# WISDEM/RAFT

Hardware: AMD Instinct MI355X
Metric: design-case-frequency solves/sec (whole node) (higher is better)
Workload: dtype f64

## Files before the change

### raft_amd/csrc/raftx_geom.h

```cpp
#pragma once

#define MP_N 24
#define MH_N 48
#define MI_N 48

__host__ __device__ inline void derive_design_tables(const double *strips, int64_t i0, int64_t i1, double *dsv,
                                                     int *dsf) {
    int64_t s = i0;
    while (s < i1) {
        int64_t e = s + 1;
        double proj[64];
        int np = 0;
        while (e < i1 && (e - s) < 64) {
            const double *pr = strips + (size_t)(e - 1) * NF, *cr = strips + (size_t)e * NF;
            bool same = true;
            double dv[3], pj = 0.0;
            for (int j = 0; j < 3; j++) {
                same = same && (pr[RAFTX_F_Q + j] == cr[RAFTX_F_Q + j]);
                dv[j] = cr[RAFTX_F_X + j] - pr[RAFTX_F_X + j];
                pj += dv[j] * cr[RAFTX_F_Q + j];
            }
            if (!same || !(pj > 0.0) || !(fabs(pj) <= 1.797e308)) break;
            double perp2 = 0.0, scale = 1.0;
            for (int j = 0; j < 3; j++) {
// ... 616 lines not shown
            for (int c = 0; c < 3; c++) {
                ra[c] = rA[c] + q[c] * a[RAFTX_GS_S];
                rb[c] = rA[c] + q[c] * b[RAFTX_GS_S];
            }
            const double aD1 = circ ? a[RAFTX_GS_D] : a[RAFTX_GS_D + 1], bD1 = circ ? b[RAFTX_GS_D] : b[RAFTX_GS_D + 1];
            if (ra[2] * rb[2] <= 0) {
                const double t = (0 - ra[2]);
                double xWP = ra[0] + t * (rb[0] - ra[0]) / (rb[2] - ra[2]);
                double yWP = ra[1] + t * (rb[1] - ra[1]) / (rb[2] - ra[2]);
                const double w0 = b[RAFTX_GS_D] + t * (a[RAFTX_GS_D] - b[RAFTX_GS_D]) / (rb[2] - ra[2]);
                const double w1 = bD1 + t * (aD1 - bD1) / (rb[2] - ra[2]);
                double AWP, IxWP, IyWP;
                if (circ) {
                    AWP = (M_PI / 4) * w0 * w0;
                    IxWP = IyWP = (M_PI / 64) * w0 * w0 * w0 * w0;
                } else {
                    AWP = w0 * w1;
                    const double Ix = (1.0 / 12) * w0 * w1 * w1 * w1, Iy = (1.0 / 12) * w0 * w0 * w0 * w1;
                    IxWP = R[0][0] * Ix * R[0][0] + R[0][1] * Iy * R[0][1];
                    IyWP = R[1][0] * Ix * R[1][0] + R[1][1] * Iy * R[1][1];
                }
                const double LWP = fabs(ra[2] / cosPhi);
                double V, hc;
                geom_frustum(a[RAFTX_GS_D], aD1, w0, w1, circ, LWP, V, hc);
                double M = 0.0;
                if (circ) M = -rg * M_PI * (w0 * w0 / 32 * (2.0 + tanPhi * tanPhi) + 0.5 * (ra[2] / cosPhi) * (ra[2] / cosPhi)) * sinPhi;
                const double Fz = rg * V;
                const double ex = ra[0] - rA[0], ey = ra[1] - rA[1];
                F[2] += Fz;
                F[3] += ey * Fz;
                F[4] += -ex * Fz;
                F[3] += M * (-sinBeta);
                F[4] += M * cosBeta;
                xWP -= rA[0];
                yWP -= rA[1];
                C[2 * 6 + 2] += rg * AWP / cosPhi;
                C[2 * 6 + 3] += rg * (-AWP * yWP);
                C[2 * 6 + 4] += rg * (AWP * xWP);
                C[3 * 6 + 2] += rg * (-AWP * yWP);
                C[3 * 6 + 3] += rg * (IxWP + AWP * yWP * yWP);
                C[3 * 6 + 4] += rg * (AWP * xWP * yWP);
                C[4 * 6 + 2] += rg * (AWP * xWP);
                C[4 * 6 + 3] += rg * (AWP * xWP * yWP);
                C[4 * 6 + 4] += rg * (IyWP + AWP * xWP * xWP);
                double rc[3];
                for (int c = 0; c < 3; c++) rc[c] = ra[c] + q[c] * hc;
                C[3 * 6 + 3] += rg * V * (rc[2] - rA[2]);
                C[4 * 6 + 4] += rg * V * (rc[2] - rA[2]);
                C[3 * 6 + 5] += -rg * V * (rc[0] - rA[0]);
                C[4 * 6 + 5] += -rg * V * (rc[1] - rA[1]);
                Vt += V;
                for (int c = 0; c < 3; c++) rcV[c] += rc[c] * V;
                AWPm = AWP;
            } else if (ra[2] <= 0 && rb[2] <= 0) {
                double V, hc;
                geom_frustum(a[RAFTX_GS_D], aD1, b[RAFTX_GS_D], bD1, circ, b[RAFTX_GS_S] - a[RAFTX_GS_S], V, hc);
                double rc[3], rr[3];
                for (int c = 0; c < 3; c++) { rc[c] = ra[c] + q[c] * hc; rr[c] = rc[c] - rA[c]; }
                const double Fz = rg * V;
                F[2] += Fz;
                F[3] += rr[1] * Fz;
                F[4] += -rr[0] * Fz;
                C[3 * 6 + 3] += rg * V * rr[2];
                C[4 * 6 + 4] += rg * V * rr[2];
                C[3 * 6 + 5] += -rg * V * rr[0];
                C[4 * 6 + 5] += -rg * V * rr[1];
                Vt += V;
                for (int c = 0; c < 3; c++) rcV[c] += rc[c] * V;
            }
        }
    }
    if (geom_along(rA[2], rB[2], b[RAFTX_GS_S], L) < 0) wet++;
    double *mh = A.mhyd + (size_t)m * MH_N, *mi = A.minert + (size_t)m * MI_N;
    if (!nostatic) {
        for (int i = 0; i < 36; i++) mh[i] = C[i];
        for (int i = 0; i < 6; i++) mh[36 + i] = F[i];
        mh[42] = Vt; mh[43] = rcV[0]; mh[44] = rcV[1]; mh[45] = rcV[2]; mh[46] = AWPm; mh[47] = 0.0;
    }
    int code = 0;
    if (!nostatic) {
        GInertia J;
        geom_inertia_init(J);
        geom_load_row(gs, 0, b);
        for (int i = 1; i < n; i++) {
#pragma unroll
            for (int f = 0; f < RAFTX_GS_N; f++) a[f] = b[f];
            geom_load_row(gs, i, b);
            geom_inertia_section(J, a, b, circ, rho_shell, trim, 0.0, rA, q, p1, p2);
        }
        const int ncap = A.capOff ? (int)(co1 - co0) : 0;
        const double *gc = A.capOff ? A.caps + (size_t)co0 * RAFTX_GC_N : nullptr;
        code = geom_inertia_caps_finish(J, gs, n, gc, ncap, circ, rho_shell, rA, q, p1, p2, A.g, mi);
    }
    double *mp = A.mpose + (size_t)m * MP_N;
    for (int i = 0; i < 3; i++) {
        mp[i] = rA0[i]; mp[3 + i] = rA[i]; mp[6 + i] = q[i]; mp[9 + i] = p1[i]; mp[12 + i] = p2[i];
    }
    mp[15] = R[0][0]; mp[16] = R[0][1]; mp[17] = R[1][0]; mp[18] = R[1][1]; mp[19] = L;
    const int wetm = ((flags & RAFTX_GM_FLAG_MCF) && circ && !(flags & RAFTX_GM_FLAG_POTMOD)) ? wet : 0;
    A.cnt[m] = wet;
    A.cntm[m] = wetm;
    if (wet) atomicAdd(reinterpret_cast<unsigned long long *>(A.off + d + 1), (unsigned long long)wet);
    if (wetm) atomicAdd(reinterpret_cast<unsigned long long *>(A.cmoff + d + 1), (unsigned long long)wetm);
    if (nostatic) {
        for (int i = 0; i < MH_N; i++) mh[i] = 0.0;
        for (int i = 0; i < MI_N; i++) mi[i] = 0.0;
        return;
    }
    if (code) {
        for (int i = 0; i < MI_N; i++) mi[i] = 0.0;
        atomicCAS(A.err, 0, (int)(m + 1));
    }
}

__global__ void k_geom_trim(GeomArgs A) {
    GEOM_NOFMA
    if (A.err[2] | A.err[3]) return;
    const int d = blockIdx.x * blockDim.x + threadIdx.x;
    if (d >= A.nDesign) return;
    double mass = A.M0[(size_t)d * 36], V = 0.0, vol = 0.0;
    for (int64_t m = A.mo(d); m < A.mo(d + 1); m++) {
        mass += A.minert[(size_t)m * MI_N + 36];
        vol += A.minert[(size_t)m * MI_N + 47];
        V += A.mhyd[(size_t)m * MH_N + 42];
    }
    if (!(vol > 0.0)) {
        A.drho[d] = 0.0;
        atomicCAS(A.err + 1, 0, d + 1);
        return;
    }
    const double sumFz = -mass * A.g + V * A.rho * A.g + (A.Fz ? A.Fz[d] : 0.0);
    A.drho[d] = sumFz / A.g / vol;
}
__global__ __launch_bounds__(128) void k_geom_reinertia(GeomArgs A) {
    GEOM_NOFMA
    if (A.err[2] | A.err[3]) return;
    const int64_t m = geom_member_of_thread(A);
    if (m < 0) return;
    const double *gm = A.gm + (size_t)m * RAFTX_GM_N;
    if ((int)gm[RAFTX_GM_FLAGS] & RAFTX_GM_FLAG_NOSTATIC) return;
    const double *gs = A.gs + (size_t)A.so(m) * RAFTX_GS_N;
    const int n = (int)(A.so(m + 1) - A.so(m));
    const double *mp = A.mpose + (size_t)m * MP_N;
    const int ncap = A.capOff ? (int)(A.co(m + 1) - A.co(m)) : 0;
    const double *gc = A.capOff ? A.caps + (size_t)A.co(m) * RAFTX_GC_N : nullptr;
    double *mi = A.minert + (size_t)m * MI_N;
    if (geom_member_inertia(gm, gs, n, gc, ncap, mp + 3, mp + 6, mp + 9, mp + 12, A.g, true, A.drho[A.mdesign[m]], mi))
        for (int i = 0; i < MI_N; i++) mi[i] = 0.0;
}

#define GSCAN_CH 4096
template <int T>
__global__ __launch_bounds__(T) void k_geom_scan_t(GeomArgs A) {
    __shared__ long long part[2][17];
    __shared__ unsigned buf[2][GSCAN_CH];
    const int t = threadIdx.x;
    const int n = A.nDesign;
    constexpr int PER = GSCAN_CH / T;
    long long carrya = 0, carryb = 0, mx = 0;
    for (int c0 = 0; c0 < n; c0 += GSCAN_CH) {
        const int cn = (n - c0 < GSCAN_CH) ? n - c0 : GSCAN_CH;
        for (int i = t; i < GSCAN_CH; i += T) {
            long long va = 0, vb = 0;
            if (i < cn) { va = A.off[c0 + i + 1]; vb = A.cmoff[c0 + i + 1]; }
            buf[0][i] = (unsigned)va;
            buf[1][i] = (unsigned)vb;
            mx = va > mx ? va : mx;
        }
        __syncthreads();
        long long a = 0, b = 0;
        for (int i = 0; i < PER; i++) { a += buf[0][t * PER + i]; b += buf[1][t * PER + i]; }
        const int lane = t & 63, wv = t >> 6;
        long long ia = a, ib = b;
        for (int o = 1; o < 64; o <<= 1) {
            const long long ua = __shfl_up(ia, o, 64), ub = __shfl_up(ib, o, 64);
            if (lane >= o) { ia += ua; ib += ub; }
        }
        if (lane == 63) { part[0][wv] = ia; part[1][wv] = ib; }
        __syncthreads();
        long long ra = carrya, rb = carryb, sa = 0, sb = 0;
        for (int i = 0; i < T / 64; i++) {
            if (i < wv) { ra += part[0][i]; rb += part[1][i]; }
            sa += part[0][i]; sb += part[1][i];
        }
        ra += ia - a;
        rb += ib - b;
        for (int i = 0; i < PER; i++) {
            ra += buf[0][t * PER + i];
            rb += buf[1][t * PER + i];
            buf[0][t * PER + i] = (unsigned)ra;
            buf[1][t * PER + i] = (unsigned)rb;
        }
        __syncthreads();
        for (int i = t; i < cn; i += T) {
            const long long va = buf[0][i], vb = buf[1][i];
            A.off[c0 + i + 1] = va;
            A.cmoff[c0 + i + 1] = vb;
            if (A.hostOut) A.hostOut[8 + c0 + i + 1] = va;
        }
        carrya += sa;
        carryb += sb;
        __syncthreads();
    }
    if (mx) atomicMax(reinterpret_cast<unsigned long long *>(A.tot + 2), (unsigned long long)mx);
    __syncthreads();
    if (t == 0) {
        A.off[0] = 0;
        A.cmoff[0] = 0;
        A.tot[0] = carrya;
        A.tot[1] = carryb;
        if (A.hostOut) {
            A.hostOut[0] = carrya;
            A.hostOut[1] = carryb;
            A.hostOut[2] = A.tot[2];
            int *e = reinterpret_cast<int *>(A.hostOut + 3);
            e[0] = A.err[0]; e[1] = A.err[1]; e[2] = A.err[2]; e[3] = A.err[3];
            A.hostOut[8] = 0;
        }
    }
}
__global__ __launch_bounds__(64) void k_geom_mcf(GeomArgs A, int64_t nRows) {
    GEOM_NOFMA
    const int64_t row = blockIdx.x;
    const int iw = blockIdx.y * blockDim.x + threadIdx.x;
    if (row >= nRows || iw >= A.nw) return;
    const double R = A.mcfaux[row * 3], Ca1 = A.mcfaux[row * 3 + 1], Ca2 = A.mcfaux[row * 3 + 2];
    const double k = A.k[iw];
    const double Tr = M_PI / 5 / R;
    double ramp;
    if (k <= 0.0) ramp = 0.0;
    else if (k < Tr) ramp = 0.5 * (1 - cos(M_PI * k / Tr));
    else ramp = 1.0;
    double cr = 0.0, ci = 0.0;
    if (ramp != 0.0) {
        const double x = k * R;
        const double hr = 0.5 * (j0(x) - jn(2, x)), hi = 0.5 * (y0(x) - yn(2, x));
        const double den = M_PI * (x * x);
        const double mag = den * (hr * hr + hi * hi);
        cr = 4.0 * hi / mag;
        ci = 4.0 * hr / mag;
    }
    A.cm[((size_t)row * 2 + 0) * A.nw + iw] = cplx{cr * ramp + (1.0 + Ca1) * (1 - ramp), ci * ramp};
    A.cm[((size_t)row * 2 + 1) * A.nw + iw] = cplx{cr * ramp + (1.0 + Ca2) * (1 - ramp), ci * ramp};
}


__device__ inline void geom_reduce_matrix(const double *C, const double (&a)[3], double *out) {
    GEOM_NOFMA
    const double H[3][3] = {{0, a[2], -a[1]}, {-a[2], 0, a[0]}, {a[1], -a[0], 0}};
    double t12[3][3], t21[3][3];
    for (int i = 0; i < 3; i++)
        for (int j = 0; j < 3; j++) {
            double s12 = C[i * 6 + 3 + j], s21 = C[(3 + i) * 6 + j];
            for (int l = 0; l < 3; l++) {
                s12 += C[i * 6 + l] * H[l][j];
                s21 += H[l][i] * C[l * 6 + j];
            }
            t12[i][j] = s12;
            t21[i][j] = s21;
        }
    for (int i = 0; i < 3; i++)
        for (int j = 0; j < 3; j++) {
            out[i * 6 + j] += C[i * 6 + j];
            out[i * 6 + 3 + j] += t12[i][j];
            out[(3 + i) * 6 + j] += t21[i][j];
            double s = C[(3 + i) * 6 + 3 + j];
            for (int l = 0; l < 3; l++) s += H[l][i] * t12[l][j] + C[(3 + i) * 6 + l] * H[l][j];
            out[(3 + i) * 6 + 3 + j] += s;
        }
}
__device__ inline void geom_reduce_vector(const double *W, const double (&a)[3], const double *arm0, const double (&th)[3],
                                          double *Wout, double *Cout) {
    GEOM_NOFMA
    Wout[0] += W[0]; Wout[1] += W[1]; Wout[2] += W[2];
    Wout[3] += W[3] + (a[1] * W[2] - a[2] * W[1]);
    Wout[4] += W[4] + (a[2] * W[0] - a[0] * W[2]);
    Wout[5] += W[5] + (a[0] * W[1] - a[1] * W[0]);
    for (int j = 0; j < 3; j++) {
        double tj[3] = {th[0], th[1], th[2]};
        tj[j] += 1.0;
        const double dA[3] = {arm0[0] + (tj[1] * a[2] - tj[2] * a[1]) - a[0], arm0[1] + (tj[2] * a[0] - tj[0] * a[2]) - a[1],
                              arm0[2] + (tj[0] * a[1] - tj[1] * a[0]) - a[2]};
        Cout[3 * 6 + 3 + j] -= dA[1] * W[2] - dA[2] * W[1];
        Cout[4 * 6 + 3 + j] -= dA[2] * W[0] - dA[0] * W[2];
        Cout[5 * 6 + 3 + j] -= dA[0] * W[1] - dA[1] * W[0];
    }
}

__device__ constexpr int DS_SRC[DS_N] = {
    -1, -1, RAFTX_F_MCF, -1,
    RAFTX_F_X, RAFTX_F_X + 1, RAFTX_F_X + 2,
    -2, -3, -4,
    RAFTX_F_AX, RAFTX_F_AX + 1, RAFTX_F_AX + 2,
    RAFTX_F_Q, RAFTX_F_Q + 1, RAFTX_F_Q + 2,
    RAFTX_F_P1, RAFTX_F_P1 + 1, RAFTX_F_P1 + 2,
    RAFTX_F_P2, RAFTX_F_P2 + 1, RAFTX_F_P2 + 2,
    RAFTX_F_IQ, RAFTX_F_IP1, RAFTX_F_IP2, RAFTX_F_AI, RAFTX_F_RHOV,
    RAFTX_F_DQ, RAFTX_F_DP1, RAFTX_F_DP2, RAFTX_F_DEND, -1};
static_assert(DS_MCF == 2 && DS_X == 4 && DS_U == 7 && DS_A == 10 && DS_Q == 13 && DS_P1 == 16 && DS_P2 == 19 &&
              DS_IQ == 22 && DS_DQ == 27 && DS_N == 32, "DS_SRC follows the device record layout");
#define GD_ROW (NF + 1)
#define GD_GM_N 3
#define GD_MP_N 13
#ifdef GEOM_PHASE_TIMING
__device__ unsigned long long geom_phase_cycles[10];
#define GEOM_PHASE(i)                                                                                   \
    do {                                                                                                \
        __syncthreads();                                                                                \
        const unsigned long long now_ = wall_clock64();                                                 \
        if (threadIdx.x == 0) atomicAdd(&geom_phase_cycles[i], now_ - tphase_);                         \
        tphase_ = now_;                                                                                 \
    } while (0)
#define GEOM_PHASE_BEGIN unsigned long long tphase_ = wall_clock64();
#else
#define GEOM_PHASE(i)
#define GEOM_PHASE_BEGIN
#endif
#ifndef GD_T
#define GD_T 128
#endif
static_assert(GD_T % 64 == 0 && GD_T % DS_N == 0 && GD_T <= 256, "k_geom_design: whole wavefronts, a lane keeps its record field");
template <bool ABI, bool ADDUP>
__device__ __forceinline__ void geom_design_block(const GeomArgs &A, const int d, double *gd_lds, int *wcnt) {
    GEOM_NOFMA
    const int lane = threadIdx.x;
    const int64_t i0 = A.off[d], i1 = A.off[d + 1];
    const int S = (int)(i1 - i0);
    double *rec = gd_lds;
    double *pjv = rec + (size_t)S * GD_ROW, *unv = pjv + S;
    int *okv = reinterpret_cast<int *>(unv + S), *rsv = okv + S, *mfl = rsv + S;
    GEOM_PHASE_BEGIN
    {
        const int64_t m0 = A.mo(d), m1 = A.mo(d + 1);
        const int nMem = (int)(m1 - m0);
        const int64_t s0 = A.so(m0);
        const int nSta = (int)(A.so(m1) - s0);
        int *mcum = mfl + S;
        int *mbase = mcum + nSta + 2 * nMem;
        int *ssta = mbase + nMem + 1;
        double *sgm = reinterpret_cast<double *>(okv + (((int)(ssta - okv) + nMem + 2) & ~1));
        double *sgs = sgm + (size_t)nMem * GD_GM_N;
        double *smp = sgs + (size_t)nSta * RAFTX_GS_N;
        {
            const double *g0 = A.gm + (size_t)m0 * RAFTX_GM_N, *g1 = A.gs + (size_t)s0 * RAFTX_GS_N, *g2 = A.mpose + (size_t)m0 * MP_N;
            const int n0 = nMem * GD_GM_N, n01 = n0 + nSta * RAFTX_GS_N, total = n01 + nMem * GD_MP_N;
            constexpr int SU = 10;
            const int64_t so_lane = lane <= nMem ? A.so(m0 + lane) : s0;
            for (int base = 0; base < total; base += SU * GD_T) {
                double v[SU];
#pragma unroll
                for (int u = 0; u < SU; u++) {
                    const int idx = base + u * GD_T + lane;
                    const double *src;
                    if (idx < n0) {
                        const int row = idx / GD_GM_N, col = idx % GD_GM_N;
                        src = g0 + (size_t)row * RAFTX_GM_N + (col == 0 ? RAFTX_GM_DLSMAX : (col == 1 ? RAFTX_GM_SHAPE : RAFTX_GM_FLAGS));
                    } else if (idx < n01) {
                        src = g1 + (idx - n0);
                    } else {
                        const int k = idx - n01, row = k / GD_MP_N, col = k % GD_MP_N;
                        src = g2 + (size_t)row * MP_N + (col < 12 ? 3 + col : 19);
                    }
                    v[u] = idx < total ? *src : 0.0;
                }
#pragma unroll
                for (int u = 0; u < SU; u++) {
                    const int idx = base + u * GD_T + lane;
                    if (idx < total) sgm[idx] = v[u];
                }
            }
            if (lane <= nMem) mbase[lane] = ssta[lane] = (int)(so_lane - s0);
            for (int mi = lane + GD_T; mi <= nMem; mi += GD_T) mbase[mi] = ssta[mi] = (int)(A.so(m0 + mi) - s0);
        }
        __syncthreads();
        for (int u = lane; u < nSta + nMem; u += GD_T) {
            int mi = 0;
            while (mi + 1 < nMem && mbase[mi + 1] + mi + 1 <= u) mi++;
            const int sta0 = mbase[mi], n = mbase[mi + 1] - sta0, g = u - (sta0 + mi);
            int cntg = 1;
            if (g > 0 && g < n) {
                const double *gs = sgs + (size_t)sta0 * RAFTX_GS_N;
                cntg = geom_interval_strips(gs[(size_t)g * RAFTX_GS_N + RAFTX_GS_S] - gs[(size_t)(g - 1) * RAFTX_GS_N + RAFTX_GS_S],
                                            sgm[(size_t)mi * GD_GM_N]);
            }
            mcum[sta0 + 2 * mi + g + 1] = cntg;
        }
        __syncthreads();
        for (int mi = lane; mi < nMem; mi += GD_T) {
            const int n = ssta[mi + 1] - ssta[mi];
            int *cum = mcum + ssta[mi] + 2 * mi;
            int a = 0;
            cum[0] = 0;
            for (int g = 0; g <= n; g++) { a += cum[g + 1]; cum[g + 1] = a; }
            mbase[mi + 1] = a;
        }
        __syncthreads();
        if (lane == 0) {
            int a = 0;
            mbase[0] = 0;
            for (int mi = 0; mi < nMem; mi++) { a += mbase[mi + 1]; mbase[mi + 1] = a; }
        }
        __syncthreads();
        const int total = mbase[nMem];
        GEOM_PHASE(0);
        const double rho = A.rho, cdrag = sqrt(8 / M_PI);
        double rP[3] = {0, 0, 0};
        if (A.pose)
            for (int i = 0; i < 3; i++) rP[i] = A.pose[(size_t)d * 6 + i];
        int nwet = 0;
        for (int t0 = 0; t0 < total; t0 += GD_T) {
            const int t = t0 + lane;
            const bool act = t < total;
            const int tq = act ? t : 0;
            int mi = 0;
            while (mi + 1 < nMem && mbase[mi + 1] <= tq) mi++;
            const int64_t m = m0 + mi;
            const int tt = tq - mbase[mi];
            const int n = ssta[mi + 1] - ssta[mi];
            const int *cum = mcum + ssta[mi] + 2 * mi;
            const double *gm = sgm + (size_t)mi * GD_GM_N;
            const double *gs = sgs + (size_t)ssta[mi] * RAFTX_GS_N;
            const double *mp = smp + (size_t)mi * GD_MP_N;
            const bool circ = gm[1] != 0.0;
            const int flags = (int)gm[2];
            const bool potMod = flags & RAFTX_GM_FLAG_POTMOD;
            const bool mcf = (flags & RAFTX_GM_FLAG_MCF) && circ && !potMod;
            const double L = mp[12];
            double rA[3], rB[3], q[3], p1[3], p2[3], armN[3];
            for (int i = 0; i < 3; i++) {
                rA[i] = mp[i]; q[i] = mp[3 + i]; p1[i] = mp[6 + i]; p2[i] = mp[9 + i];
                rB[i] = rA[i] + L * q[i];
                armN[i] = rA[i] - rP[i];
            }
            int g = 0;
            while (g < n && cum[g + 1] <= tt) g++;
            const int j = tt - cum[g];
            const int nsub = (g > 0 && g < n) ? cum[g + 1] - cum[g] : 1;
            GStrip st = geom_strip(gs, n, g, j, nsub, circ);
            double r[3];
            for (int c = 0; c < 3; c++) r[c] = geom_along(rA[c], rB[c], st.ls, L);
            const bool wet = act && (r[2] < 0);
            const GLocate at = geom_locate(st.ls, gs, n);
            const unsigned long long mask = __ballot(wet);
            const int wv = lane >> 6, ln = lane & 63;
            if (ln == 0) wcnt[wv] = __popcll(mask);
            __syncthreads();
            int before = 0, all = 0;
            for (int w = 0; w < GD_T / 64; w++) {
                before += w < wv ? wcnt[w] : 0;
                all += wcnt[w];
            }
            const int pos = nwet + before + __popcll(mask & ((1ull << ln) - 1ull));
            nwet += all;
            __syncthreads();
            if (!wet || pos >= S) continue;
            double *row = rec + (size_t)pos * GD_ROW;
            for (int c = 0; c < NF; c++) row[c] = 0.0;
            for (int c = 0; c < 3; c++) {
                row[RAFTX_F_X + c] = r[c];
                row[RAFTX_F_AX + c] = (r[c] - rA[c]) + armN[c];
                row[RAFTX_F_Q + c] = q[c];
                row[RAFTX_F_P1 + c] = p1[c];
                row[RAFTX_F_P2 + c] = p2[c];
            }
            row[RAFTX_F_CIRC] = circ ? 1.0 : 0.0;
            row[RAFTX_F_MCF] = -1.0;
            row[26] = (double)mi;
            row[27] = (double)tt;
            const double ds0 = st.ds0, ds1 = st.ds1, dr0 = st.drs0, dr1 = st.drs1, dls = st.dls;
            if (!potMod) {
                double v_i, v_end, a_i;
                if (circ) {
                    v_i = 0.25 * M_PI * ds0 * ds0 * dls;
                    const double a3 = ds0 + dr0, b3 = ds0 - dr0;
                    v_end = M_PI / 12.0 * fabs(a3 * a3 * a3 - b3 * b3 * b3);
                    a_i = M_PI * ds0 * dr0;
                } else {
                    v_i = ds0 * ds1 * dls;
                    const double ma = 0.5 * ((ds0 + dr0) + (ds1 + dr1)), mb = 0.5 * ((ds0 - dr0) + (ds1 - dr1));
                    v_end = M_PI / 12.0 * (ma * ma * ma - mb * mb * mb);
                    a_i = (ds0 + dr0) * (ds1 + dr1) - (ds0 - dr0) * (ds1 - dr1);
                }
                if (r[2] + 0.5 * dls > 0) v_i = v_i * (0.5 * dls - r[2]) / dls;
                const double Ca1 = geom_interp_at(at, st.ls, gs, RAFTX_GS_CA + 1), Ca2 = geom_interp_at(at, st.ls, gs, RAFTX_GS_CA + 2);
                const double CaE = geom_interp_at(at, st.ls, gs, RAFTX_GS_CA + 3);
                row[RAFTX_F_IQ] = rho * v_end * CaE;
                row[RAFTX_F_AI] = a_i;
                row[RAFTX_F_RHOV] = rho * v_i;
                row[RAFTX_F_AP1] = rho * v_i * Ca1;
                row[RAFTX_F_AP2] = rho * v_i * Ca2;
                if (mcf) {
                    int64_t cmbase = A.cmoff[d], cmrow0 = cmbase;
                    int wet0 = 0;
                    for (int64_t mm = m0; mm < m; mm++) { cmrow0 += A.cntm[mm]; wet0 += A.cnt[mm]; }
                    const int posm = pos - wet0;
                    row[RAFTX_F_MCF] = (double)((cmrow0 - cmbase) + posm);
                    double *ax = A.mcfaux + (size_t)(cmrow0 + posm) * 3;
                    ax[0] = ds0 / 2; ax[1] = Ca1; ax[2] = Ca2;
                } else {
                    row[RAFTX_F_IP1] = rho * v_i * (1.0 + Ca1);
                    row[RAFTX_F_IP2] = rho * v_i * (1.0 + Ca2);
                }
            }
            double a_q, a_p1, a_p2, a_end;
            if (circ) {
                a_q = M_PI * ds0 * dls; a_p1 = ds0 * dls; a_p2 = ds0 * dls; a_end = fabs(M_PI * ds0 * dr0);
            } else {
                a_q = 2 * (ds0 + ds0) * dls; a_p1 = ds0 * dls; a_p2 = ds1 * dls;
                a_end = fabs((ds0 + dr0) * (ds1 + dr1) - (ds0 - dr0) * (ds1 - dr1));
            }
            row[RAFTX_F_DQ] = cdrag * 0.5 * rho * a_q * geom_interp_at(at, st.ls, gs, RAFTX_GS_CD + 0);
            row[RAFTX_F_DP1] = cdrag * 0.5 * rho * a_p1 * geom_interp_at(at, st.ls, gs, RAFTX_GS_CD + 1);
            row[RAFTX_F_DP2] = cdrag * 0.5 * rho * a_p2 * geom_interp_at(at, st.ls, gs, RAFTX_GS_CD + 2);
            row[RAFTX_F_DEND] = cdrag * 0.5 * rho * a_end * geom_interp_at(at, st.ls, gs, RAFTX_GS_CD + 3);
        }
        __syncthreads();
        GEOM_PHASE(1);
        if constexpr (ABI) {
            double *abi = A.abi + (size_t)i0 * NF;
            for (int t = lane; t < S * NF; t += GD_T) abi[t] = rec[(t / NF) * GD_ROW + (t % NF)];
        }
    }
    __syncthreads();
    GEOM_PHASE(2);
    for (int t = lane; t < S; t += GD_T) {
        bool pass = false;
        double pj = 0.0;
        const double *pr = rec + (size_t)(t > 0 ? t - 1 : 0) * GD_ROW, *cr = rec + (size_t)t * GD_ROW;
        double pq[3], cq[3], px[3], cx[3];
        for (int j = 0; j < 3; j++) {
            pq[j] = pr[RAFTX_F_Q + j]; cq[j] = cr[RAFTX_F_Q + j]; px[j] = pr[RAFTX_F_X + j]; cx[j] = cr[RAFTX_F_X + j];
        }
        if (t > 0) {
            bool same = true;
            double dv[3];
            for (int j = 0; j < 3; j++) {
                same = same && (pq[j] == cq[j]);
                dv[j] = cx[j] - px[j];
                pj += dv[j] * cq[j];
            }
            if (same && (pj > 0.0) && (fabs(pj) <= 1.797e308)) {
                double perp2 = 0.0, scale = 1.0;
                for (int j = 0; j < 3; j++) {
                    double tt = dv[j] - pj * cq[j];
                    perp2 += tt * tt;
                    scale += fabs(cx[j]);
                }
                pass = !(sqrt(perp2) > 1e-10 * scale);
            }
        }
        okv[t] = pass ? 1 : 0;
        pjv[t] = pj;
    }
    __syncthreads();
    bool serial = S > GD_T;
    if (!serial) {
        const int wv = lane >> 6, ln = lane & 63;
        const bool st = lane < S && (lane == 0 || !okv[lane]);
        const unsigned long long mask = __ballot(st);
        if (ln == 0) wcnt[wv] = mask ? wv * 64 + 63 - __builtin_clzll(mask) : -1;
        if (st) reinterpret_cast<unsigned long long *>(unv)[lane] = 0x7ff0000000000000ull;
        __syncthreads();
        const unsigned long long below = mask & (ln == 63 ? ~0ull : ((2ull << ln) - 1ull));
        int s = below ? wv * 64 + 63 - __builtin_clzll(below) : -1;
        for (int w = wv - 1; w >= 0 && s < 0; w--) s = wcnt[w];
        if (lane < S) {
            rsv[lane] = s;
            if (!st) atomicMin(reinterpret_cast<unsigned long long *>(unv) + s, (unsigned long long)__double_as_longlong(pjv[lane]));
        }
        serial = __syncthreads_or(lane < S && lane - s >= 64) != 0;
        if (!serial && st && reinterpret_cast<unsigned long long *>(unv)[lane] == 0x7ff0000000000000ull) unv[lane] = 0.0;
    }
    if (serial && lane == 0) {
        int s = 0;
        double unit = 0.0;
        for (int t = 0; t < S; t++) {
            if (t == 0 || !okv[t] || (t - s) >= 64) {
                if (t > 0) unv[s] = unit;
                s = t;
                unit = 0.0;
            } else {
                const double pj = pjv[t];
                unit = (unit == 0.0 || pj < unit) ? pj : unit;
            }
            rsv[t] = s;
        }
        if (S > 0) unv[s] = unit;
    }
    __syncthreads();
    for (int t = lane; t < S; t += GD_T) {
        const int s = rsv[t];
        const double unit = unv[s];
        const double *cr = rec + (size_t)t * GD_ROW, *pr = rec + (size_t)(t > 0 ? t - 1 : 0) * GD_ROW;
        double cX[3], cQ[3], cP1[3], cP2[3], cA[3], pX[3], pP1[3], pP2[3], pA[3];
        for (int j = 0; j < 3; j++) {
            cX[j] = cr[RAFTX_F_X + j]; cQ[j] = cr[RAFTX_F_Q + j]; cP1[j] = cr[RAFTX_F_P1 + j]; cP2[j] = cr[RAFTX_F_P2 + j];
            cA[j] = cr[RAFTX_F_AX + j];
            pX[j] = pr[RAFTX_F_X + j]; pP1[j] = pr[RAFTX_F_P1 + j]; pP2[j] = pr[RAFTX_F_P2 + j]; pA[j] = pr[RAFTX_F_AX + j];
        }
        const double cCirc = cr[RAFTX_F_CIRC], cMcf = cr[RAFTX_F_MCF], pCirc = pr[RAFTX_F_CIRC], pMcf = pr[RAFTX_F_MCF];
        const double pjt = pjv[t];
        int m = 0;
        if (t > s && unit > 0.0) {
            double ratio = pjt / unit;
            int mi = (int)floor(ratio + 0.5);
            if (mi >= 1 && mi <= 2 && fabs(ratio - mi) < 1e-9) {
                bool ok = true;
                for (int j = 0; j < 3; j++) {
                    double pred = pX[j] + (double)mi * unit * cQ[j];
                    if (fabs(pred - cX[j]) > 1e-10 * (1.0 + fabs(cX[j]))) ok = false;
                }
                if (ok) m = mi;
            }
        }
        if (m != 0) {
            for (int j = 0; j < 3; j++)
                if (pP1[j] != cP1[j] || pP2[j] != cP2[j]) m = 0;
            if ((pCirc != 0.0) != (cCirc != 0.0)) m = 0;
            if ((pMcf >= 0.0) != (cMcf >= 0.0)) m = 0;
            for (int j = 0; j < 3; j++) {
                const double da = cA[j] - pA[j], dx = cX[j] - pX[j];
                if (!(fabs(da - dx) <= 1e-9 * (1.0 + fabs(cX[j]) + fabs(cA[j])))) m = 0;
            }
        }
        int fl = m | (cCirc != 0.0 ? DSI_CIRC : 0);
        if (fabs(cP1[0]) < 1e-15 && fabs(cP1[1]) < 1e-15 && fabs(cP2[2]) < 1e-15) fl |= DSI_AXAL;
        if (fabs(cQ[0]) < 1e-15 && fabs(cQ[1]) < 1e-15 && fabs(cP1[2]) < 1e-15 && fabs(cP2[2]) < 1e-15)
            fl |= DSI_VAX;
        A.dsi[(size_t)i0 + t] = fl;
    }
    GEOM_PHASE(3);
    {
        double *dso = A.ds + (size_t)i0 * DS_N;
        const int j = lane % DS_N, f = DS_SRC[j], nT = S * DS_N;
        constexpr int DU = 4;
        for (int t0 = lane; t0 < nT; t0 += DU * GD_T) {
          double vv[DU];
#pragma unroll
          for (int u = 0; u < DU; u++) {
            const int t = t0 + u * GD_T;
            const int i = t < nT ? t / DS_N : 0;
            const double *cr = rec + (size_t)i * GD_ROW;
            double v = 0.0;
            if (f >= 0) v = cr[f];
            else if (f <= -2) v = unv[rsv[i]] * cr[RAFTX_F_Q + (-2 - f)];
            if (t < nT && j == DS_MCF && v >= 0.0) {
                const double *ax0 = A.mcfaux + (size_t)A.cmoff[d] * 3, *axm = ax0 + (size_t)v * 3;
                const int mrow = (int)v;
                for (int r = 0; r < mrow; r++)
                    if (ax0[r * 3] == axm[0] && ax0[r * 3 + 1] == axm[1] && ax0[r * 3 + 2] == axm[2]) {
                        v = (double)r;
                        break;
                    }
            }
            vv[u] = v;
          }
#pragma unroll
          for (int u = 0; u < DU; u++) {
            const int t = t0 + u * GD_T;
            if (t < nT) dso[t] = vv[u];
          }
        }
    }
    GEOM_PHASE(4);
    constexpr int GV = 21;
    for (int t0 = 0; t0 < S; t0 += GD_T) {
        const int t = t0 + lane;
        double gv[GV];
        if (t < S) {
            const double *cr = rec + (size_t)t * GD_ROW;
            const double ax = cr[RAFTX_F_AX], ay = cr[RAFTX_F_AX + 1], az = cr[RAFTX_F_AX + 2];
            const double cs[3] = {cr[RAFTX_F_AP1], cr[RAFTX_F_AP2], cr[RAFTX_F_IQ]};
            const int fs[3] = {RAFTX_F_P1, RAFTX_F_P2, RAFTX_F_Q};
            for (int tt = 0; tt < 3; tt++) {
                const double nx = cr[fs[tt]], ny = cr[fs[tt] + 1], nz = cr[fs[tt] + 2];
                gv[tt * 7] = cs[tt];
                gv[tt * 7 + 1] = nx; gv[tt * 7 + 2] = ny; gv[tt * 7 + 3] = nz;
                gv[tt * 7 + 4] = ay * nz - az * ny;
                gv[tt * 7 + 5] = az * nx - ax * nz;
                gv[tt * 7 + 6] = ax * ny - ay * nx;
            }
        }
        __syncthreads();
        if (t < S)
            for (int e = 0; e < GV; e++) rec[(size_t)t * GV + e] = gv[e];
    }
    __syncthreads();
    GEOM_PHASE(5);
    {
        const int k3 = lane / 36, e = lane % 36, i = e / 6, j = e % 6;
        double am = 0.0;
        if (k3 < 3) {
            const int lo = (int)(((long long)S * k3) / 3), hi = (int)(((long long)S * (k3 + 1)) / 3);
            for (int s = lo; s < hi; s++) {
                const double *g = rec + (size_t)s * GV;
                for (int tt = 0; tt < 3; tt++) am += g[tt * 7] * g[tt * 7 + 1 + i] * g[tt * 7 + 1 + j];
            }
        }
        __syncthreads();
        if (k3 < 3) rec[lane] = am;
        __syncthreads();
        if (lane < 36) {
            am = (rec[lane] + rec[36 + lane]) + rec[72 + lane];
            const size_t o = (size_t)d * 36 + lane;
            A.A[o] = am;
            if constexpr (ADDUP) {
                double m0 = A.M0[o], c0 = A.C0[o];
                if (A.add_mask & RAFTX_ADD_MORISON) m0 += am;
                if (A.add_mask & RAFTX_ADD_HYDROSTATIC) c0 += A.Ch[o];
                if (A.add_mask & RAFTX_ADD_INERTIA) { m0 += A.Ms[o]; c0 += A.Cs[o]; }
                A.M0[o] = m0;
                A.C0[o] = c0;
            }
        }
    }
    GEOM_PHASE(6);
    (void)mfl;
}
__global__ __launch_bounds__(GD_T) void k_geom_design(GeomArgs A) {
    extern __shared__ double gd_lds[];
    __shared__ int wcnt[GD_T / 64];
    if ((int)blockIdx.x >= A.nDesign) return;
    if (A.abi) geom_design_block<true, false>(A, (int)blockIdx.x, gd_lds, wcnt);
    else if (A.addup_in_design) geom_design_block<false, true>(A, (int)blockIdx.x, gd_lds, wcnt);
    else geom_design_block<false, false>(A, (int)blockIdx.x, gd_lds, wcnt);
}
__global__ void k_geom_addup(GeomArgs A) {
    const size_t o = (size_t)blockIdx.x * blockDim.x + threadIdx.x;
    if (o >= (size_t)A.nDesign * 36) return;
    if (A.add_mask & RAFTX_ADD_MORISON) A.M0[o] += A.A[o];
    if (A.add_mask & RAFTX_ADD_HYDROSTATIC) A.C0[o] += A.Ch[o];
    if (A.add_mask & RAFTX_ADD_INERTIA) { A.M0[o] += A.Ms[o]; A.C0[o] += A.Cs[o]; }
}
static size_t geom_design_lds(int maxS, int maxSta, int maxMem) {
    const size_t S = (size_t)(maxS > 0 ? maxS : 1);
    return sizeof(double) * (S * GD_ROW + 2 * S) + sizeof(int) * (3 * S + (size_t)maxSta + 3 * (size_t)maxMem + 1) + 16 +
           sizeof(int) * ((size_t)maxMem + 4) +
           sizeof(double) * ((size_t)maxMem * (GD_GM_N + GD_MP_N) + (size_t)maxSta * RAFTX_GS_N);
}

__global__ __launch_bounds__(64) void k_geom_reduce(GeomArgs A) {
    GEOM_NOFMA
    const int t = blockIdx.x * blockDim.x + threadIdx.x;
    const int d = t / 3, role = t % 3;
    if (d >= A.nDesign) return;
    double th[3] = {0, 0, 0}, rP[3] = {0, 0, 0};
    if (A.pose)
        for (int i = 0; i < 3; i++) { rP[i] = A.pose[(size_t)d * 6 + i]; th[i] = A.pose[(size_t)d * 6 + 3 + i]; }
    double out[36], Wv[6] = {0, 0, 0, 0, 0, 0}, sc0 = 0.0, sc1 = 0.0, sr[3] = {0, 0, 0};
    for (int i = 0; i < 36; i++) out[i] = 0.0;
    for (int64_t m = A.mo(d); m < A.mo(d + 1); m++) {
        const double *mp = A.mpose + (size_t)m * MP_N, *mh = A.mhyd + (size_t)m * MH_N, *mi = A.minert + (size_t)m * MI_N;
        const double a[3] = {mp[3] - rP[0], mp[4] - rP[1], mp[5] - rP[2]};
        double C[36];
        if (role == 1) {
            for (int i = 0; i < 36; i++) C[i] = 0.0;
            C[3 * 6 + 3] = C[4 * 6 + 4] = mi[46];
        } else {
            const double *src = role == 0 ? mh : mi;
            for (int i = 0; i < 36; i++) C[i] = src[i];
        }
        geom_reduce_matrix(C, a, out);
        if (role < 2) {
            const double *W = role == 0 ? mh + 36 : mi + 40;
            geom_reduce_vector(W, a, mp, th, Wv, out);
        }
        if (role == 2) {
            for (int c = 0; c < 3; c++) sr[c] += ((mi[37 + c] - mp[3 + c]) + mp[c]) * mi[36];
            sc0 += mi[47];
        } else if (role == 0) {
            const double V = mh[42];
            sc0 += V;
            sc1 += mh[46];
            if (V > 0)
                for (int c = 0; c < 3; c++) sr[c] += ((mh[43 + c] / V - mp[3 + c]) + mp[c]) * V;
        }
    }
    for (int i = 0; i < 6; i++)
        for (int j = i + 1; j < 6; j++) {
            const double s = (out[i * 6 + j] + out[j * 6 + i]) / 2;
            out[i * 6 + j] = out[j * 6 + i] = s;
        }
    double *dst = (role == 0 ? A.Ch : role == 1 ? A.Cs : A.Ms) + (size_t)d * 36;
    for (int i = 0; i < 36; i++) dst[i] = out[i];
    double *pr = A.props + (size_t)d * RAFTX_SP_N;
    if (role == 0) {
        for (int i = 0; i < 6; i++) A.Wh[(size_t)d * 6 + i] = Wv[i];
        pr[RAFTX_SP_V] = sc0;
        pr[RAFTX_SP_AWP] = sc1;
        for (int c = 0; c < 3; c++) pr[RAFTX_SP_RCB + c] = sc0 != 0.0 ? sr[c] / sc0 : 0.0;
    } else if (role == 1) {
        for (int i = 0; i < 6; i++) A.Ws[(size_t)d * 6 + i] = Wv[i];
    } else {
        pr[RAFTX_SP_VFILL] = sc0;
        pr[RAFTX_SP_DRHO] = (A.add_mask & RAFTX_TRIM_BALLAST) ? A.drho[d] : 0.0;
        pr[RAFTX_SP_MASS] = out[0];
        for (int c = 0; c < 3; c++) pr[RAFTX_SP_RCG + c] = out[0] != 0.0 ? sr[c] / out[0] : 0.0;
        pr[11] = 0.0;
    }
}

struct ExpandArgs {
    int n, nM, nSt, nCap, nP;
    const double *params;
    const double *gm, *gs, *gc;
    const int *stMember, *capMember;
    const double *stFrac, *fillFrac, *capFrac;
    const double *endCoef, *headCS, *diaCoef;
    const int *endEdit, *diaEdit;
    double *gm_out, *gs_out, *gc_out;
};
__device__ inline double affine_eval(const double *coef, const double *p, int nP) {
    GEOM_NOFMA
    double v = coef[0];
    for (int q = 0; q < nP; q++) v = v + coef[1 + q] * p[q];
    return v;
}
// ... 68 lines not shown
```

Before: 678.5 million.

## Use a wavefront prefix scan for strip counts and branchless group lookup in geom design

The three serial passes that built per-member cumulative strip counts (per-element count, per-member scan, single-thread member scan) are replaced by one wavefront that computes counts and does a shuffle-based inclusive scan over a flat group-start array. Linear while-loop searches for member and sub-interval are replaced by unrolled, branchless 8-way counting searches. The per-round wet-count buffer is double-buffered so the second barrier in each strip round can be dropped. Row writes are deferred to a single store pass with no zero-fill, and debug columns are only written when ABI output is needed. This cuts barriers and serial scans in exchange for more involved indexing. There is a risk that fields no longer zeroed, such as 26, 27, STEP and UNIT in non-ABI mode, are read later.

```diff
diff --git a/raft_amd/csrc/raftx_geom.h b/raft_amd/csrc/raftx_geom.h
--- a/raft_amd/csrc/raftx_geom.h
+++ b/raft_amd/csrc/raftx_geom.h
@@ -942,6 +942,34 @@
 #define GD_ROW (NF + 1)
 #define GD_GM_N 3
 #define GD_MP_N 13
+__device__ __forceinline__ int geom_group_member(const int *ssta, int nMem, int u) {
+    int mi = 0;
+    for (int k0 = 1; k0 < nMem; k0 += 8) {
+        int sv[8];
+#pragma unroll
+        for (int k = 0; k < 8; k++) sv[k] = ssta[min(k0 + k, nMem - 1)];
+#pragma unroll
+        for (int k = 0; k < 8; k++) mi += (k0 + k < nMem && sv[k] + k0 + k <= u) ? 1 : 0;
+    }
+    return mi;
+}
+__device__ __forceinline__ int geom_find_group(const int *gst, int nG, int t) {
+    const int stride = (nG + 7) >> 3;
+    int sv[8], b = 0;
+#pragma unroll
+    for (int k = 1; k < 8; k++) sv[k] = gst[min(k * stride, nG)];
+#pragma unroll
+    for (int k = 1; k < 8; k++) b += sv[k] <= t ? 1 : 0;
+    const int base = b * stride;
+    int u = base;
+    for (int i0 = 1; i0 < stride; i0 += 8) {
+#pragma unroll
+        for (int k = 0; k < 8; k++) sv[k] = gst[min(base + i0 + k, nG)];
+#pragma unroll
+        for (int k = 0; k < 8; k++) u += (i0 + k < stride && sv[k] <= t) ? 1 : 0;
+    }
+    return u;
+}
 #ifdef GEOM_PHASE_TIMING
 __device__ unsigned long long geom_phase_cycles[10];
 #define GEOM_PHASE(i)                                                                                   \
@@ -975,9 +1003,9 @@
         const int nMem = (int)(m1 - m0);
         const int64_t s0 = A.so(m0);
         const int nSta = (int)(A.so(m1) - s0);
-        int *mcum = mfl + S;
-        int *mbase = mcum + nSta + 2 * nMem;
-        int *ssta = mbase + nMem + 1;
+        const int nG = nSta + nMem;
+        int *gst = mfl + S;
+        int *ssta = gst + nSta + 3 * nMem + 1;
         double *sgm = reinterpret_cast<double *>(okv + (((int)(ssta - okv) + nMem + 2) & ~1));
         double *sgs = sgm + (size_t)nMem * GD_GM_N;
         double *smp = sgs + (size_t)nSta * RAFTX_GS_N;
@@ -1009,39 +1037,38 @@
                     if (idx < total) sgm[idx] = v[u];
                 }
             }
-            if (lane <= nMem) mbase[lane] = ssta[lane] = (int)(so_lane - s0);
-            for (int mi = lane + GD_T; mi <= nMem; mi += GD_T) mbase[mi] = ssta[mi] = (int)(A.so(m0 + mi) - s0);
+            if (lane <= nMem) ssta[lane] = (int)(so_lane - s0);
+            for (int mi = lane + GD_T; mi <= nMem; mi += GD_T) ssta[mi] = (int)(A.so(m0 + mi) - s0);
         }
         __syncthreads();
-        for (int u = lane; u < nSta + nMem; u += GD_T) {
-            int mi = 0;
-            while (mi + 1 < nMem && mbase[mi + 1] + mi + 1 <= u) mi++;
-            const int sta0 = mbase[mi], n = mbase[mi + 1] - sta0, g = u - (sta0 + mi);
-            int cntg = 1;
-            if (g > 0 && g < n) {
-                const double *gs = sgs + (size_t)sta0 * RAFTX_GS_N;
-                cntg = geom_interval_strips(gs[(size_t)g * RAFTX_GS_N + RAFTX_GS_S] - gs[(size_t)(g - 1) * RAFTX_GS_N + RAFTX_GS_S],
-                                            sgm[(size_t)mi * GD_GM_N]);
-            }
-            mcum[sta0 + 2 * mi + g + 1] = cntg;
+        if (lane < 64) {
+            int carry = 0;
+            for (int u0 = 0; u0 < nG; u0 += 64) {
+                const int u = u0 + lane;
+                int cntg = 0;
+                if (u < nG) {
+                    const int mi = geom_group_member(ssta, nMem, u);
+                    const int sta0 = ssta[mi], n = ssta[mi + 1] - sta0, g = u - (sta0 + mi);
+                    cntg = 1;
+                    if (g > 0 && g < n) {
+                        const double *gs = sgs + (size_t)sta0 * RAFTX_GS_N;
+                        cntg = geom_interval_strips(gs[(size_t)g * RAFTX_GS_N + RAFTX_GS_S] - gs[(size_t)(g - 1) * RAFTX_GS_N + RAFTX_GS_S],
+                                                    sgm[(size_t)mi * GD_GM_N]);
+                    }
+                }
+                int inc = cntg;
+#pragma unroll
+                for (int o = 1; o < 64; o <<= 1) {
+                    const int below = __shfl_up(inc, o);
+                    if (lane >= o) inc += below;
+                }
+                if (u < nG) gst[u + 1] = carry + inc;
+                carry += __shfl(inc, 63);
+            }
+            if (lane == 0) gst[0] = 0;
         }
         __syncthreads();
-        for (int mi = lane; mi < nMem; mi += GD_T) {
-            const int n = ssta[mi + 1] - ssta[mi];
-            int *cum = mcum + ssta[mi] + 2 * mi;
-            int a = 0;
-            cum[0] = 0;
-            for (int g = 0; g <= n; g++) { a += cum[g + 1]; cum[g + 1] = a; }
-            mbase[mi + 1] = a;
-        }
-        __syncthreads();
-        if (lane == 0) {
-            int a = 0;
-            mbase[0] = 0;
-            for (int mi = 0; mi < nMem; mi++) { a += mbase[mi + 1]; mbase[mi + 1] = a; }
-        }
-        __syncthreads();
-        const int total = mbase[nMem];
+        const int total = gst[nG];
         GEOM_PHASE(0);
         const double rho = A.rho, cdrag = sqrt(8 / M_PI);
         double rP[3] = {0, 0, 0};
@@ -1052,14 +1079,14 @@
             const int t = t0 + lane;
             const bool act = t < total;
             const int tq = act ? t : 0;
-            int mi = 0;
-            while (mi + 1 < nMem && mbase[mi + 1] <= tq) mi++;
+            const int u = geom_find_group(gst, nG, tq);
+            const int mi = geom_group_member(ssta, nMem, u);
             const int64_t m = m0 + mi;
-            const int tt = tq - mbase[mi];
-            const int n = ssta[mi + 1] - ssta[mi];
-            const int *cum = mcum + ssta[mi] + 2 * mi;
+            const int sta0 = ssta[mi], n = ssta[mi + 1] - sta0, g = u - (sta0 + mi);
+            const int first = gst[u], j = tq - first;
+            const int nsub = (g > 0 && g < n) ? gst[u + 1] - first : 1;
             const double *gm = sgm + (size_t)mi * GD_GM_N;
-            const double *gs = sgs + (size_t)ssta[mi] * RAFTX_GS_N;
+            const double *gs = sgs + (size_t)sta0 * RAFTX_GS_N;
             const double *mp = smp + (size_t)mi * GD_MP_N;
             const bool circ = gm[1] != 0.0;
             const int flags = (int)gm[2];
@@ -1072,10 +1099,6 @@
                 rB[i] = rA[i] + L * q[i];
                 armN[i] = rA[i] - rP[i];
             }
-            int g = 0;
-            while (g < n && cum[g + 1] <= tt) g++;
-            const int j = tt - cum[g];
-            const int nsub = (g > 0 && g < n) ? cum[g + 1] - cum[g] : 1;
             GStrip st = geom_strip(gs, n, g, j, nsub, circ);
             double r[3];
             for (int c = 0; c < 3; c++) r[c] = geom_along(rA[c], rB[c], st.ls, L);
@@ -1083,30 +1106,19 @@
             const GLocate at = geom_locate(st.ls, gs, n);
             const unsigned long long mask = __ballot(wet);
             const int wv = lane >> 6, ln = lane & 63;
-            if (ln == 0) wcnt[wv] = __popcll(mask);
+            unsigned char *wround = reinterpret_cast<unsigned char *>(wcnt) + ((t0 / GD_T) & 1) * (GD_T / 64);
+            if (ln == 0) wround[wv] = (unsigned char)__popcll(mask);
             __syncthreads();
             int before = 0, all = 0;
             for (int w = 0; w < GD_T / 64; w++) {
-                before += w < wv ? wcnt[w] : 0;
-                all += wcnt[w];
+                const int cw = wround[w];
+                before += w < wv ? cw : 0;
+                all += cw;
             }
             const int pos = nwet + before + __popcll(mask & ((1ull << ln) - 1ull));
             nwet += all;
-            __syncthreads();
             if (!wet || pos >= S) continue;
-            double *row = rec + (size_t)pos * GD_ROW;
-            for (int c = 0; c < NF; c++) row[c] = 0.0;
-            for (int c = 0; c < 3; c++) {
-                row[RAFTX_F_X + c] = r[c];
-                row[RAFTX_F_AX + c] = (r[c] - rA[c]) + armN[c];
-                row[RAFTX_F_Q + c] = q[c];
-                row[RAFTX_F_P1 + c] = p1[c];
-                row[RAFTX_F_P2 + c] = p2[c];
-            }
-            row[RAFTX_F_CIRC] = circ ? 1.0 : 0.0;
-            row[RAFTX_F_MCF] = -1.0;
-            row[26] = (double)mi;
-            row[27] = (double)tt;
+            double fIq = 0.0, fIp1 = 0.0, fIp2 = 0.0, fAi = 0.0, fRhov = 0.0, fAp1 = 0.0, fAp2 = 0.0, fMcf = -1.0;
             const double ds0 = st.ds0, ds1 = st.ds1, dr0 = st.drs0, dr1 = st.drs1, dls = st.dls;
             if (!potMod) {
                 double v_i, v_end, a_i;
@@ -1124,22 +1136,22 @@
                 if (r[2] + 0.5 * dls > 0) v_i = v_i * (0.5 * dls - r[2]) / dls;
                 const double Ca1 = geom_interp_at(at, st.ls, gs, RAFTX_GS_CA + 1), Ca2 = geom_interp_at(at, st.ls, gs, RAFTX_GS_CA + 2);
                 const double CaE = geom_interp_at(at, st.ls, gs, RAFTX_GS_CA + 3);
-                row[RAFTX_F_IQ] = rho * v_end * CaE;
-                row[RAFTX_F_AI] = a_i;
-                row[RAFTX_F_RHOV] = rho * v_i;
-                row[RAFTX_F_AP1] = rho * v_i * Ca1;
-                row[RAFTX_F_AP2] = rho * v_i * Ca2;
+                fIq = rho * v_end * CaE;
+                fAi = a_i;
+                fRhov = rho * v_i;
+                fAp1 = rho * v_i * Ca1;
+                fAp2 = rho * v_i * Ca2;
                 if (mcf) {
                     int64_t cmbase = A.cmoff[d], cmrow0 = cmbase;
                     int wet0 = 0;
                     for (int64_t mm = m0; mm < m; mm++) { cmrow0 += A.cntm[mm]; wet0 += A.cnt[mm]; }
                     const int posm = pos - wet0;
-                    row[RAFTX_F_MCF] = (double)((cmrow0 - cmbase) + posm);
+                    fMcf = (double)((cmrow0 - cmbase) + posm);
                     double *ax = A.mcfaux + (size_t)(cmrow0 + posm) * 3;
                     ax[0] = ds0 / 2; ax[1] = Ca1; ax[2] = Ca2;
                 } else {
-                    row[RAFTX_F_IP1] = rho * v_i * (1.0 + Ca1);
-                    row[RAFTX_F_IP2] = rho * v_i * (1.0 + Ca2);
+                    fIp1 = rho * v_i * (1.0 + Ca1);
+                    fIp2 = rho * v_i * (1.0 + Ca2);
                 }
             }
             double a_q, a_p1, a_p2, a_end;
@@ -1149,10 +1161,37 @@
                 a_q = 2 * (ds0 + ds0) * dls; a_p1 = ds0 * dls; a_p2 = ds1 * dls;
                 a_end = fabs((ds0 + dr0) * (ds1 + dr1) - (ds0 - dr0) * (ds1 - dr1));
             }
-            row[RAFTX_F_DQ] = cdrag * 0.5 * rho * a_q * geom_interp_at(at, st.ls, gs, RAFTX_GS_CD + 0);
-            row[RAFTX_F_DP1] = cdrag * 0.5 * rho * a_p1 * geom_interp_at(at, st.ls, gs, RAFTX_GS_CD + 1);
-            row[RAFTX_F_DP2] = cdrag * 0.5 * rho * a_p2 * geom_interp_at(at, st.ls, gs, RAFTX_GS_CD + 2);
-            row[RAFTX_F_DEND] = cdrag * 0.5 * rho * a_end * geom_interp_at(at, st.ls, gs, RAFTX_GS_CD + 3);
+            const double fDq = cdrag * 0.5 * rho * a_q * geom_interp_at(at, st.ls, gs, RAFTX_GS_CD + 0);
+            const double fDp1 = cdrag * 0.5 * rho * a_p1 * geom_interp_at(at, st.ls, gs, RAFTX_GS_CD + 1);
+            const double fDp2 = cdrag * 0.5 * rho * a_p2 * geom_interp_at(at, st.ls, gs, RAFTX_GS_CD + 2);
+            const double fDend = cdrag * 0.5 * rho * a_end * geom_interp_at(at, st.ls, gs, RAFTX_GS_CD + 3);
+            double *row = rec + (size_t)pos * GD_ROW;
+            for (int c = 0; c < 3; c++) {
+                row[RAFTX_F_X + c] = r[c];
+                row[RAFTX_F_AX + c] = (r[c] - rA[c]) + armN[c];
+                row[RAFTX_F_Q + c] = q[c];
+                row[RAFTX_F_P1 + c] = p1[c];
+                row[RAFTX_F_P2 + c] = p2[c];
+            }
+            row[RAFTX_F_IQ] = fIq;
+            row[RAFTX_F_IP1] = fIp1;
+            row[RAFTX_F_IP2] = fIp2;
+            row[RAFTX_F_AI] = fAi;
+            row[RAFTX_F_DQ] = fDq;
+            row[RAFTX_F_DP1] = fDp1;
+            row[RAFTX_F_DP2] = fDp2;
+            row[RAFTX_F_DEND] = fDend;
+            row[RAFTX_F_CIRC] = circ ? 1.0 : 0.0;
+            row[RAFTX_F_MCF] = fMcf;
+            row[RAFTX_F_RHOV] = fRhov;
+            if constexpr (ABI) {
+                row[26] = (double)mi;
+                row[27] = (double)(tq - gst[sta0 + mi]);
+                row[RAFTX_F_STEP] = 0.0;
+                row[RAFTX_F_UNIT] = 0.0;
+            }
+            row[RAFTX_F_AP1] = fAp1;
+            row[RAFTX_F_AP2] = fAp2;
         }
         __syncthreads();
         GEOM_PHASE(1);
```

Result: no change. 684.0 million (median of 6 runs) (+0.8%).
